# pythoncrazy/jimm

Hardware: NVIDIA H100
Metric: images/sec (higher is better)
Workload: dtype f16

## Files before the change

jimm_b200/csrc/common.cuh:

```cuda
#pragma once

#include <cuda.h>
#include <cuda_bf16.h>
#include <cuda_fp16.h>
#include <cuda_fp8.h>
#include <cuda_runtime.h>
#include <stdint.h>

#include <atomic>
#include <mutex>
#include <string>

namespace jimm {

void set_last_error(const char* fmt, ...);

#define JIMM_CUDA_CHECK(expr)                                                                   \
  do {                                                                                          \
    cudaError_t _e = (expr);                                                                    \
    if (_e != cudaSuccess) {                                                                    \
      ::jimm::set_last_error("%s:%d: %s -> %s", __FILE__, __LINE__, #expr, cudaGetErrorString(_e)); \
      return -2;                                                                                \
    }                                                                                           \
  } while (0)
// ... 80 lines not shown
      : "=r"(pred));
  return pred != 0;
}

__device__ __forceinline__ void mbar_init(uint64_t* bar, uint32_t count) {
  asm volatile("mbarrier.init.shared::cta.b64 [%0], %1;" ::"r"(smem_u32(bar)), "r"(count));
}
__device__ __forceinline__ void fence_barrier_init() {
  asm volatile("fence.mbarrier_init.release.cluster;" ::: "memory");
}
__device__ __forceinline__ void fence_proxy_async_smem() {
  asm volatile("fence.proxy.async.shared::cta;" ::: "memory");
}
__device__ __forceinline__ void mbar_arrive(uint64_t* bar) {
  asm volatile("mbarrier.arrive.shared::cta.b64 _, [%0];" ::"r"(smem_u32(bar)) : "memory");
}
__device__ __forceinline__ void mbar_arrive_expect_tx(uint64_t* bar, uint32_t bytes) {
  asm volatile("mbarrier.arrive.expect_tx.shared::cta.b64 _, [%0], %1;" ::"r"(smem_u32(bar)), "r"(bytes) : "memory");
}
__device__ __forceinline__ void mbar_wait(uint64_t* bar, uint32_t parity) {
  asm volatile(
      "{\n\t.reg .pred P1;\n\t"
      "WAIT_LOOP:\n\t"
      "mbarrier.try_wait.parity.shared::cta.b64 P1, [%0], %1;\n\t"
      "@P1 bra DONE;\n\t"
      "bra WAIT_LOOP;\n\t"
      "DONE:\n\t}" ::"r"(smem_u32(bar)),
      "r"(parity)
      : "memory");
}

__device__ __forceinline__ bool mbar_test_wait(uint64_t* bar, uint32_t parity) {
  uint32_t ok;
  asm volatile(
      "{\n\t.reg .pred P1;\n\t"
      "mbarrier.test_wait.parity.shared::cta.b64 P1, [%1], %2;\n\t"
      "selp.u32 %0, 1, 0, P1;\n\t}"
      : "=r"(ok)
      : "r"(smem_u32(bar)), "r"(parity)
      : "memory");
  return ok != 0;
}

__device__ __forceinline__ void tma_prefetch_desc(const CUtensorMap* m) {
  asm volatile("prefetch.tensormap [%0];" ::"l"(reinterpret_cast<uint64_t>(m)) : "memory");
}
__device__ __forceinline__ void tma_load_2d(void* smem_dst, const CUtensorMap* m, uint64_t* bar, int c0, int c1) {
  asm volatile(
      "cp.async.bulk.tensor.2d.shared::cluster.global.mbarrier::complete_tx::bytes [%0], [%1, {%3, %4}], [%2];" ::"r"(
          smem_u32(smem_dst)),
      "l"(reinterpret_cast<uint64_t>(m)), "r"(smem_u32(bar)), "r"(c0), "r"(c1)
      : "memory");
}

__device__ __forceinline__ void tma_store_2d(const CUtensorMap* m, uint32_t smem_src, int c0, int c1) {
  asm volatile("cp.async.bulk.tensor.2d.global.shared::cta.bulk_group [%0, {%2, %3}], [%1];" ::"l"(reinterpret_cast<uint64_t>(m)),
               "r"(smem_src), "r"(c0), "r"(c1)
               : "memory");
}
__device__ __forceinline__ void tma_reduce_add_2d(const CUtensorMap* m, uint32_t smem_src, int c0, int c1) {
  asm volatile("cp.reduce.async.bulk.tensor.2d.global.shared::cta.add.tile.bulk_group [%0, {%2, %3}], [%1];" ::"l"(
                   reinterpret_cast<uint64_t>(m)),
               "r"(smem_src), "r"(c0), "r"(c1)
               : "memory");
}
__device__ __forceinline__ void tma_store_3d(const CUtensorMap* m, uint32_t smem_src, int c0, int c1, int c2) {
  asm volatile("cp.async.bulk.tensor.3d.global.shared::cta.bulk_group [%0, {%2, %3, %4}], [%1];" ::"l"(reinterpret_cast<uint64_t>(m)),
               "r"(smem_src), "r"(c0), "r"(c1), "r"(c2)
               : "memory");
}
__device__ __forceinline__ void tma_reduce_add_3d(const CUtensorMap* m, uint32_t smem_src, int c0, int c1, int c2) {
  asm volatile("cp.reduce.async.bulk.tensor.3d.global.shared::cta.add.tile.bulk_group [%0, {%2, %3, %4}], [%1];" ::"l"(
                   reinterpret_cast<uint64_t>(m)),
               "r"(smem_src), "r"(c0), "r"(c1), "r"(c2)
               : "memory");
}
__device__ __forceinline__ void tma_store_commit() { asm volatile("cp.async.bulk.commit_group;" ::: "memory"); }
__device__ __forceinline__ void tma_store_wait_read() { asm volatile("cp.async.bulk.wait_group.read 0;" ::: "memory"); }
__device__ __forceinline__ void tma_store_wait_read1() { asm volatile("cp.async.bulk.wait_group.read 1;" ::: "memory"); }
__device__ __forceinline__ void tma_store_wait_all() { asm volatile("cp.async.bulk.wait_group 0;" ::: "memory"); }

__device__ __forceinline__ uint32_t cluster_ctarank() {
  uint32_t r;
  asm volatile("mov.u32 %0, %%cluster_ctarank;" : "=r"(r));
  return r;
}
__device__ __forceinline__ void cluster_sync_all() {
  asm volatile("barrier.cluster.arrive.release.aligned;\n\tbarrier.cluster.wait.acquire.aligned;" ::: "memory");
}
__device__ __forceinline__ uint32_t mapa_shared(uint32_t local_smem_addr, uint32_t rank) {
  uint32_t r;
  asm volatile("mapa.shared::cluster.u32 %0, %1, %2;" : "=r"(r) : "r"(local_smem_addr), "r"(rank));
  return r;
}
__device__ __forceinline__ void mbar_arrive_cluster(uint32_t cluster_addr) {
  asm volatile("mbarrier.arrive.release.cluster.shared::cluster.b64 _, [%0];" ::"r"(cluster_addr) : "memory");
}
__device__ __forceinline__ uint64_t make_wgmma_desc_sw128(uint32_t smem_addr) {
  uint64_t d = 0;
  d |= static_cast<uint64_t>((smem_addr & 0x3FFFFu) >> 4);
  d |= static_cast<uint64_t>(1) << 16;
  d |= static_cast<uint64_t>(1024 >> 4) << 32;
  d |= static_cast<uint64_t>(1) << 62;
  return d;
}
template <int SW>
__device__ __forceinline__ uint64_t make_wgmma_desc(uint32_t smem_addr, uint32_t lbo) {
  static_assert(SW == 128 || SW == 64 || SW == 32, "swizzle width");
  constexpr uint64_t layout = SW == 128 ? 1 : SW == 64 ? 2 : 3;
  uint64_t d = 0;
  d |= static_cast<uint64_t>((smem_addr & 0x3FFFFu) >> 4);
  d |= static_cast<uint64_t>((lbo >> 4) & 0x3FFFu) << 16;
  d |= static_cast<uint64_t>(8 * SW >> 4) << 32;
  d |= layout << 62;
  return d;
}
__device__ __forceinline__ void wgmma_fence() { asm volatile("wgmma.fence.sync.aligned;" ::: "memory"); }
__device__ __forceinline__ void wgmma_commit() { asm volatile("wgmma.commit_group.sync.aligned;" ::: "memory"); }
template <int N>
__device__ __forceinline__ void wgmma_wait() { asm volatile("wgmma.wait_group.sync.aligned %0;" ::"n"(N) : "memory"); }
template <int R>
__device__ __forceinline__ void wgmma_fence_operands(float (&d)[R]) {
#pragma unroll
  for (int i = 0; i < R; ++i) asm volatile("" : "+f"(d[i])::"memory");
}

#define JIMM_WGMMA_D128                                                                                                                    \
  "{%0, %1, %2, %3, %4, %5, %6, %7, %8, %9, %10, %11, %12, %13, %14, %15, %16, %17, %18, %19, %20, %21, %22, %23, %24, %25, %26, %27, "     \
  "%28, %29, %30, %31, %32, %33, %34, %35, %36, %37, %38, %39, %40, %41, %42, %43, %44, %45, %46, %47, %48, %49, %50, %51, %52, %53, %54, " \
  "%55, %56, %57, %58, %59, %60, %61, %62, %63, %64, %65, %66, %67, %68, %69, %70, %71, %72, %73, %74, %75, %76, %77, %78, %79, %80, %81, " \
  "%82, %83, %84, %85, %86, %87, %88, %89, %90, %91, %92, %93, %94, %95, %96, %97, %98, %99, %100, %101, %102, %103, %104, %105, %106, "   \
  "%107, %108, %109, %110, %111, %112, %113, %114, %115, %116, %117, %118, %119, %120, %121, %122, %123, %124, %125, %126, %127}"
#define JIMM_WGMMA_D8(i) "+f"(d[i]), "+f"(d[i + 1]), "+f"(d[i + 2]), "+f"(d[i + 3]), "+f"(d[i + 4]), "+f"(d[i + 5]), "+f"(d[i + 6]), "+f"(d[i + 7])
#define JIMM_WGMMA_D128_OPERANDS                                                                                                 \
  JIMM_WGMMA_D8(0), JIMM_WGMMA_D8(8), JIMM_WGMMA_D8(16), JIMM_WGMMA_D8(24), JIMM_WGMMA_D8(32), JIMM_WGMMA_D8(40), JIMM_WGMMA_D8(48), \
      JIMM_WGMMA_D8(56), JIMM_WGMMA_D8(64), JIMM_WGMMA_D8(72), JIMM_WGMMA_D8(80), JIMM_WGMMA_D8(88), JIMM_WGMMA_D8(96),             \
      JIMM_WGMMA_D8(104), JIMM_WGMMA_D8(112), JIMM_WGMMA_D8(120)
template <int KIND>
__device__ __forceinline__ void wgmma_m64n256_ss(float (&d)[128], uint64_t adesc, uint64_t bdesc, uint32_t accumulate) {
  if constexpr (KIND == 0) {
    asm volatile("{\n\t.reg .pred p;\n\tsetp.ne.b32 p, %130, 0;\n\t"
                 "wgmma.mma_async.sync.aligned.m64n256k16.f32.f16.f16 " JIMM_WGMMA_D128 ", %128, %129, p, 1, 1, 0, 0;\n\t}"
                 : JIMM_WGMMA_D128_OPERANDS
                 : "l"(adesc), "l"(bdesc), "r"(accumulate));
  } else if constexpr (KIND == 1) {
    asm volatile("{\n\t.reg .pred p;\n\tsetp.ne.b32 p, %130, 0;\n\t"
                 "wgmma.mma_async.sync.aligned.m64n256k16.f32.bf16.bf16 " JIMM_WGMMA_D128 ", %128, %129, p, 1, 1, 0, 0;\n\t}"
                 : JIMM_WGMMA_D128_OPERANDS
                 : "l"(adesc), "l"(bdesc), "r"(accumulate));
// ... 260 lines not shown
```

jimm_b200/csrc/gemm.cu:

```cuda
#include "gemm.cuh"

#include <stdarg.h>
#include <stdio.h>
#include <stdlib.h>
#include <string.h>

#include <type_traits>

#include "common.cuh"

namespace jimm {

static constexpr int BM = GEMM_TILE_M;
static constexpr int BN = GEMM_TILE_N;
static_assert(BM == 128 && BN == 256, "the warp roles and the wgmma shape below are written for 128 x 256 tiles");
static constexpr int STAGES = 4;
static constexpr int A_STAGE_BYTES = BM * 128;
static constexpr int B_STAGE_BYTES = BN * 128;
static constexpr int STAGE_BYTES = A_STAGE_BYTES + B_STAGE_BYTES;
static constexpr int EPI_WARPS = 8;
static constexpr int EPI_BOX_ROWS = 16;
static constexpr int EPI_BUF_BYTES = EPI_BOX_ROWS * 128;
static constexpr int EPI_BUFS = 2;
static constexpr int EPI_STAGE_BYTES = EPI_WARPS * EPI_BUFS * EPI_BUF_BYTES;
// ... 257 lines not shown
        *reinterpret_cast<float2*>(p1) = make_float2(v2, v3);
      }
    }
    fence_proxy_async_smem();
    __syncwarp();
    if (lane == 0) {
      const uint32_t tbuf_u32 = smem_u32(tbuf);
      if constexpr (OUT == OUT_F32_ADD) {
        if (epi.tok_pad > 0) {
          const int b = row_base / epi.tok_pad;
          tma_reduce_add_3d(map_c, tbuf_u32, n0, row_base - b * epi.tok_pad + epi.tok_off, b);
        } else {
          tma_reduce_add_2d(map_c, tbuf_u32, n0, row_base);
        }
      } else {
        tma_store_2d(map_c, tbuf_u32, n0, row_base);
      }
      tma_store_commit();
    }
  }
}

template <bool SCALED, int NC>
__device__ __forceinline__ void epilogue_generic(const EpiDev& epi, const float (&acc)[NC / 2], int lane, int row_base, int n_tile0) {
  const int g = lane >> 2, t = lane & 3;
#pragma unroll
  for (int h = 0; h < 2; ++h) {
    const int row = row_base + g + 8 * h;
    if (row >= epi.M) continue;
    int out_row, add_row;
    remap_row(epi, row, out_row, add_row);
    float sa = 1.f;
    if constexpr (SCALED) sa = __ldg(epi.a_scale + row);
#pragma unroll
    for (int j = 0; j < NC / 8; ++j) {
#pragma unroll
      for (int q = 0; q < 2; ++q) {
        const int col = n_tile0 + 8 * j + 2 * t + q;
        if (col < epi.N) {
          float v = acc[4 * j + 2 * h + q];
          if constexpr (SCALED) v *= sa * __ldg(epi.b_scale + col);
          if (epi.bias) v += __ldg(epi.bias + col);
          v = apply_act(v, epi.act);
          if (epi.rowadd) v += __ldg(epi.rowadd + static_cast<size_t>(add_row) * epi.N + col);
          if (epi.residual) v += epi.residual[static_cast<size_t>(out_row) * epi.ldr + col];
          store1(epi, out_row, col, v);
        }
      }
    }
  }
}


template <typename T, int OUT, int ACT>
__global__ void __launch_bounds__(NUM_THREADS, 1)
gemm_wgmma_kernel(const __grid_constant__ CUtensorMap map_a, const __grid_constant__ CUtensorMap map_b,
                  const __grid_constant__ CUtensorMap map_c, const EpiDev epi, int K) {
  constexpr bool SCALED = kScaled<T>;
  constexpr int BK = 128 / sizeof(T);
  constexpr int UK = 32 / sizeof(T);
  constexpr int TM = tile_rows(Traits<T>::DTYPE);
  constexpr int STAGE_TX = TM * 128 + B_STAGE_BYTES;
  constexpr int WG_DM = SCALED ? 0 : 64;
  constexpr int WG_DN = SCALED ? 128 : 0;
  constexpr int NC = BN - WG_DN;
  constexpr bool FUSE_LN = OUT == OUT_F32_ADD && ACT == ACT_FUSE_LN;
  constexpr int EPI_ACT = ACT == ACT_FUSE_LN ? static_cast<int>(ACT_NONE) : ACT;
  constexpr int PRODUCER_REGS = FUSE_LN ? 152 : 40;
  constexpr int CONSUMER_REGS = FUSE_LN ? 176 : 232;
  static_assert(128 * PRODUCER_REGS + 256 * CONSUMER_REGS <= NUM_THREADS * KERNEL_REGS, "register split exceeds the CTA's allocation");

  extern __shared__ uint8_t smem_raw[];
  uint8_t* smem = reinterpret_cast<uint8_t*>((reinterpret_cast<uintptr_t>(smem_raw) + 1023) & ~static_cast<uintptr_t>(1023));
  uint8_t* smem_a = smem;
  uint8_t* smem_b = smem + STAGES * A_STAGE_BYTES;
  uint8_t* epi_stage = smem + STAGES * STAGE_BYTES;
  LnQueue* lnq = reinterpret_cast<LnQueue*>(epi_stage + EPI_STAGE_BYTES);
  uint64_t* full_bar = reinterpret_cast<uint64_t*>(lnq + 1);
  uint64_t* empty_bar = full_bar + STAGES;

  const int warp_idx = threadIdx.x >> 5;
  const int lane = threadIdx.x & 31;
  const int M = epi.M, N = epi.N;
  const int m_tiles = (M + TM - 1) / TM, n_tiles = (N + BN - 1) / BN;
  const int num_tiles = m_tiles * n_tiles;
  const int num_kb = (K + BK - 1) / BK;

  pdl_launch_dependents();
  if (warp_idx == 0 && lane == 0) {
    tma_prefetch_desc(&map_a);
    tma_prefetch_desc(&map_b);
    if constexpr (OUT != OUT_GENERIC) tma_prefetch_desc(&map_c);
    for (int s = 0; s < STAGES; ++s) {
      mbar_init(&full_bar[s], 1);
      mbar_init(&empty_bar[s], EPI_WARPS);
    }
    fence_barrier_init();
  }
  if constexpr (FUSE_LN) {
    if (warp_idx == 1) {
      for (int i = lane; i < LNQ; i += 32) lnq->slot[i] = -1;
      if (lane == 0) lnq->head = lnq->tail = lnq->done = 0;
    }
  }
  __syncthreads();
  pdl_wait();

  if (warp_idx < 4) {
    setmaxnreg<KERNEL_REGS, PRODUCER_REGS>();
    if (warp_idx == 0) {
      if (lane == 0) {
        int stage = 0;
        uint32_t phase = 0;
        for (int tile = blockIdx.x; tile < num_tiles; tile += gridDim.x) {
          const int tv = epi.reverse ? num_tiles - 1 - tile : tile;
          const int m_blk = tv / n_tiles, n_blk = tv - m_blk * n_tiles;
          for (int kb = 0; kb < num_kb; ++kb) {
            mbar_wait(&empty_bar[stage], phase ^ 1);
            mbar_arrive_expect_tx(&full_bar[stage], STAGE_TX);
            tma_load_2d(smem_a + stage * A_STAGE_BYTES, &map_a, &full_bar[stage], kb * BK, m_blk * TM);
            tma_load_2d(smem_b + stage * B_STAGE_BYTES, &map_b, &full_bar[stage], kb * BK, n_blk * BN);
            if (++stage == STAGES) { stage = 0; phase ^= 1; }
          }
        }
      }
    } else if constexpr (FUSE_LN) {
      ln_worker<T>(epi, lnq, lane);
    }
  } else {
    setmaxnreg<KERNEL_REGS, CONSUMER_REGS>();
    const int wg = (warp_idx - 4) >> 2;
    const int wq = warp_idx & 3;
    uint8_t* tbuf0 = epi_stage + (warp_idx - 4) * EPI_BUFS * EPI_BUF_BYTES;
    int stage = 0;
    uint32_t phase = 0, box_count = 0;
    int ln_rg = -1, ln_cols = 0;
    float acc[NC / 2];
    for (int tile = blockIdx.x; tile < num_tiles; tile += gridDim.x) {
      const int tv = epi.reverse ? num_tiles - 1 - tile : tile;
      const int m_blk = tv / n_tiles, n_blk = tv - m_blk * n_tiles;
      int prev = -1;
      if constexpr (SCALED) {
#pragma unroll
        for (int i = 0; i < NC / 2; ++i) acc[i] = 0.f;
      }
      for (int kb = 0; kb < num_kb; ++kb) {
        mbar_wait(&full_bar[stage], phase);
        const uint64_t adesc = make_wgmma_desc_sw128(smem_u32(smem_a + stage * A_STAGE_BYTES + wg * WG_DM * 128));
        const uint64_t bdesc = make_wgmma_desc_sw128(smem_u32(smem_b + stage * B_STAGE_BYTES + wg * WG_DN * 128));
        if constexpr (SCALED) {
          float slab[NC / 2];
          wgmma_fence_operands(slab);
          wgmma_fence();
#pragma unroll
          for (int k = 0; k < BK / UK; ++k)
            wgmma_m64n128k32_e4m3_ss(slab, adesc + static_cast<uint64_t>(2 * k), bdesc + static_cast<uint64_t>(2 * k), k != 0 ? 1u : 0u);
          wgmma_commit();
          wgmma_wait<0>();
          wgmma_fence_operands(slab);
          if (lane == 0) mbar_arrive(&empty_bar[stage]);
#pragma unroll
          for (int i = 0; i < NC / 2; ++i) acc[i] += slab[i];
        } else {
          wgmma_fence_operands(acc);
          wgmma_fence();
#pragma unroll
          for (int k = 0; k < BK / UK; ++k)
            wgmma_m64n256_ss<Traits<T>::KIND>(acc, adesc + static_cast<uint64_t>(2 * k), bdesc + static_cast<uint64_t>(2 * k), (kb | k) != 0 ? 1u : 0u);
          wgmma_commit();
          wgmma_fence_operands(acc);
          if (prev >= 0) {
            wgmma_wait<1>();
            if (lane == 0) mbar_arrive(&empty_bar[prev]);
          }
          prev = stage;
        }
        if (++stage == STAGES) { stage = 0; phase ^= 1; }
      }
      if constexpr (!SCALED) {
        wgmma_wait<0>();
        wgmma_fence_operands(acc);
        if (lane == 0) mbar_arrive(&empty_bar[prev]);
      }

      const int row_base = m_blk * TM + wg * WG_DM + wq * 16;
      const int n_tile0 = n_blk * BN + wg * WG_DN;
      if constexpr (OUT == OUT_GENERIC) {
        epilogue_generic<SCALED, NC>(epi, acc, lane, row_base, n_tile0);
      } else {
        if (row_base < M && (WG_DN == 0 || n_tile0 < N))
          epilogue_tma<OUT, EPI_ACT, SCALED, NC>(&map_c, epi, acc, tbuf0, lane, row_base, n_tile0, box_count);
        if constexpr (FUSE_LN) {
          if (lane == 0 && ln_rg >= 0) ln_publish(epi, lnq, ln_rg, ln_cols);
          ln_rg = (row_base & ~31) < M ? row_base >> 5 : -1;
          ln_cols = min(BN, N - n_tile0);
        }
      }
    }
    if constexpr (FUSE_LN) {
      if (lane == 0) {
        if (ln_rg >= 0) ln_publish(epi, lnq, ln_rg, ln_cols);
        __threadfence_block();
        atomicAdd(&lnq->done, 1);
      }
    }
    if constexpr (OUT != OUT_GENERIC) {
      if (lane == 0) tma_store_wait_all();
    }
  }
}

template <typename T>
__global__ void gemm_simt_kernel(const T* __restrict__ A, int lda, const T* __restrict__ B, int ldb, int K, EpiDev epi) {
  __shared__ float As[16][17], Bs[16][17];
  const int tx = threadIdx.x, ty = threadIdx.y;
  const int row = blockIdx.y * 16 + ty, col = blockIdx.x * 16 + tx;
  float acc = 0.f;
  for (int k0 = 0; k0 < K; k0 += 16) {
    const int ar = blockIdx.y * 16 + ty, ak = k0 + tx;
    As[ty][tx] = (ar < epi.M && ak < K) ? to_float(A[static_cast<size_t>(ar) * lda + ak]) : 0.f;
    const int br = blockIdx.x * 16 + ty, bk = k0 + tx;
    Bs[ty][tx] = (br < epi.N && bk < K) ? to_float(B[static_cast<size_t>(br) * ldb + bk]) : 0.f;
    __syncthreads();
#pragma unroll
    for (int k = 0; k < 16; ++k) acc += As[ty][k] * Bs[tx][k];
    __syncthreads();
  }
  if (row < epi.M && col < epi.N) {
    int out_row, add_row;
    remap_row(epi, row, out_row, add_row);
    float v = acc;
    if constexpr (kScaled<T>) v *= epi.a_scale[row] * epi.b_scale[col];
    if (epi.bias) v += epi.bias[col];
    v = apply_act(v, epi.act);
    if (epi.rowadd) v += epi.rowadd[static_cast<size_t>(add_row) * epi.N + col];
    if (epi.residual) v += epi.residual[static_cast<size_t>(out_row) * epi.ldr + col];
    store1(epi, out_row, col, v);
  }
}

static constexpr int SMEM_BYTES = STAGES * STAGE_BYTES + EPI_STAGE_BYTES + static_cast<int>(sizeof(LnQueue)) + 2 * STAGES * 8 + 1024;
static_assert(SMEM_BYTES <= 232448, "exceeds 227 KB of shared memory");
typedef CUresult (*PFN_encodeTiled)(CUtensorMap*, CUtensorMapDataType, cuuint32_t, void*, const cuuint64_t*, const cuuint64_t*,
                                    const cuuint32_t*, const cuuint32_t*, CUtensorMapInterleave, CUtensorMapSwizzle,
                                    CUtensorMapL2promotion, CUtensorMapFloatOOBfill);

static PFN_encodeTiled get_encode_fn() {
  static std::atomic<PFN_encodeTiled> fn{nullptr};
  if (PFN_encodeTiled f = fn.load(std::memory_order_acquire)) return f;
  void* p = nullptr;
  cudaDriverEntryPointQueryResult qres;
  cudaError_t e = cudaGetDriverEntryPoint("cuTensorMapEncodeTiled", &p, cudaEnableDefault, &qres);
  if (e != cudaSuccess || qres != cudaDriverEntryPointSuccess || p == nullptr) {
    set_last_error("cudaGetDriverEntryPoint(cuTensorMapEncodeTiled) failed: %s", cudaGetErrorString(e));
    return nullptr;
  }
  fn.store(reinterpret_cast<PFN_encodeTiled>(p), std::memory_order_release);
  return reinterpret_cast<PFN_encodeTiled>(p);
}

static CUtensorMapDataType tensor_map_dtype(int dtype) {
  switch (dtype) {
// ... 40 lines not shown
  return 0;
}

int device_sm_count() {
  static std::atomic<int> sms[DeviceOnce::kMaxDevices] = {};
  int dev = 0;
  cudaGetDevice(&dev);
  if (dev < 0 || dev >= DeviceOnce::kMaxDevices) dev = 0;
  int n = sms[dev].load(std::memory_order_relaxed);
  if (n == 0) {
    cudaDeviceGetAttribute(&n, cudaDevAttrMultiProcessorCount, dev);
    const char* env = getenv("JIMM_NUM_SMS");
    if (env && atoi(env) > 0) n = atoi(env);
    sms[dev].store(n, std::memory_order_relaxed);
  }
  return n;
}

static int check_epi(const GemmEpilogue& e, int N) {
  if (e.out == nullptr) { set_last_error("gemm: null output"); return -1; }
  if (e.ldo < N) { set_last_error("gemm: ldo (%d) < N (%d)", e.ldo, N); return -1; }
  return 0;
}
static int check_e4m3_epi(const GemmEpilogue& e) {
  if (e.a_scale == nullptr || e.b_scale == nullptr) { set_last_error("gemm: e4m3 operands need row scales for A and B"); return -1; }
  if ((reinterpret_cast<uintptr_t>(e.b_scale) & 7) != 0) { set_last_error("gemm: the B scales must be 8-byte aligned"); return -1; }
  if (e.residual || e.rowadd || e.rows_in != 0 || e.tok_pad != 0 || e.ln_cnt) {
    set_last_error("gemm: e4m3 operands support bias and activation epilogues only (no residual, row-add, row remap, token scatter or "
                   "fused LayerNorm)");
    return -1;
  }
  return 0;
}
int gemm_plan_init(GemmPlan* plan, int dtype, const void* A, int lda, const void* B, int ldb, int M, int N, int K,
                   const GemmEpilogue& epi) {
  if (M <= 0 || N <= 0 || K <= 0) { set_last_error("gemm: bad shape %dx%dx%d", M, N, K); return -1; }
  if (int rc = check_epi(epi, N)) return rc;
  if (dtype == DT_E4M3) {
    if (int rc = check_e4m3_epi(epi)) return rc;
  }
  if (epi.tok_pad != 0) {
    if (epi.tok_pad < 0 || epi.tok_pad % EPI_BOX_ROWS != 0 || M % epi.tok_pad != 0 || epi.tok_off < 0 || epi.tok_S <= 0) {
      set_last_error("gemm: token scatter needs tok_pad a positive multiple of %d dividing M (tok_pad=%d M=%d tok_off=%d tok_S=%d)", EPI_BOX_ROWS,
                     epi.tok_pad, M, epi.tok_off, epi.tok_S);
      return -1;
    }
    if (epi.residual != epi.out || epi.ldr != epi.ldo || epi.out_type != DT_F32) {
      set_last_error("gemm: token scatter reduce-adds into an fp32 output that is also the residual");
      return -1;
    }
  }
  if (int rc = make_tensor_map_2d(&plan->map_a, dtype, A, M, K, lda, tile_rows(dtype))) return rc;
  if (int rc = make_tensor_map_2d(&plan->map_b, dtype, B, N, K, ldb, BN)) return rc;
  plan->M = M; plan->N = N; plan->K = K; plan->dtype = dtype; plan->epi = epi;
  memset(&plan->map_c, 0, sizeof(plan->map_c));
  if (plan->epi.mode == 2) {
    const size_t es = dtype_size(epi.out_type);
    const bool ok = epi.rowadd == nullptr && epi.rows_in == 0 && (static_cast<size_t>(N) * es) % 16 == 0 &&
                    (epi.residual == nullptr || (epi.residual == epi.out && epi.ldr == epi.ldo && epi.out_type == DT_F32)) &&
                    (static_cast<size_t>(epi.ldo) * es) % 16 == 0 && (reinterpret_cast<uintptr_t>(epi.out) & 15) == 0 &&
                    (epi.bias == nullptr || ((reinterpret_cast<uintptr_t>(epi.bias) & 15) == 0 && N % 4 == 0)) &&
                    !(epi.residual && epi.act != ACT_NONE);
    if (ok && epi.tok_pad > 0) {
      if (int rc = make_tensor_map_3d(&plan->map_c, DT_F32, epi.out, M / epi.tok_pad, epi.tok_S, N, epi.ldo)) return rc;
    } else if (ok) {
      if (int rc = make_tensor_map_2d(&plan->map_c, epi.out_type, epi.out, M, N, epi.ldo, EPI_BOX_ROWS)) return rc;
    } else {
      plan->epi.mode = 0;
    }
  }
  if (epi.tok_pad > 0 && plan->epi.mode != 2) {
    set_last_error("gemm: the token scatter needs the TMA epilogue (mode 2, no activation, 16-byte aligned output / bias, N %% 4 == 0)");
    return -1;
  }
  return 0;
}

static EpiDev to_dev(const GemmEpilogue& e, int M, int N) {
  EpiDev d;
  d.bias = e.bias; d.rowadd = e.rowadd; d.residual = e.residual; d.out = e.out;
  d.act = e.act; d.ldr = e.ldr; d.out_type = e.out_type; d.ldo = e.ldo;
  d.rows_in = e.rows_in; d.rows_out = e.rows_out; d.row_off = e.row_off; d.mode = e.mode;
  d.M = M; d.N = N;
  d.tok_pad = e.tok_pad; d.tok_off = e.tok_off;
  d.reverse = e.reverse;
  d.ln_scale = e.ln_scale; d.ln_bias = e.ln_bias; d.ln_out = e.ln_out; d.ln_cnt = e.ln_cnt;
  d.ln_out_type = e.ln_out_type; d.ln_ldo = e.ln_ldo; d.ln_eps = e.ln_eps;
  d.a_scale = e.a_scale; d.b_scale = e.b_scale;
  return d;
}

template <typename T, int OUT, int ACT>
static int launch_one(const GemmPlan* p, int M, cudaStream_t stream) {
  auto* kernel = gemm_wgmma_kernel<T, OUT, ACT>;
  constexpr int TM = tile_rows(Traits<T>::DTYPE);
  static DeviceOnce attr_set;
  if (int rc = attr_set.run([&]() -> int {
        JIMM_CUDA_CHECK(cudaFuncSetAttribute(kernel, cudaFuncAttributeMaxDynamicSharedMemorySize, SMEM_BYTES));
        cudaFuncAttributes fa;
        JIMM_CUDA_CHECK(cudaFuncGetAttributes(&fa, kernel));
        if (fa.numRegs != KERNEL_REGS) {
          set_last_error("gemm: kernel compiled with %d registers per thread, the warpgroup register split assumes %d", fa.numRegs, KERNEL_REGS);
          return -2;
        }
        return 0;
      }))
    return rc;
  const int tiles = ((M + TM - 1) / TM) * ((p->N + BN - 1) / BN);
  const int grid = tiles < device_sm_count() ? tiles : device_sm_count();
  JIMM_CUDA_CHECK(launch_k(kernel, dim3(grid), dim3(NUM_THREADS), SMEM_BYTES, stream, 1, true, p->map_a, p->map_b, p->map_c,
                           to_dev(p->epi, M, p->N), p->K));
  note_launch();
  return 0;
}

template <typename T, int OUT>
static int launch_act(const GemmPlan* p, int M, cudaStream_t stream) {
  switch (p->epi.act) {
    case ACT_GELU_TANH: return launch_one<T, OUT, ACT_GELU_TANH>(p, M, stream);
    case ACT_QUICK_GELU: return launch_one<T, OUT, ACT_QUICK_GELU>(p, M, stream);
    default: return launch_one<T, OUT, ACT_NONE>(p, M, stream);
  }
}

template <typename T>
static int launch_tc(const GemmPlan* p, int M, cudaStream_t stream) {
  const GemmEpilogue& e = p->epi;
  if (e.mode != 2) return launch_one<T, OUT_GENERIC, ACT_NONE>(p, M, stream);
  if constexpr (!kScaled<T>) {
    if (e.residual) return gemm_fuses_ln(p, M) ? launch_one<T, OUT_F32_ADD, ACT_FUSE_LN>(p, M, stream) : launch_one<T, OUT_F32_ADD, ACT_NONE>(p, M, stream);
  }
  switch (e.out_type) {
    case DT_F16: return launch_act<T, OUT_H16>(p, M, stream);
    case DT_BF16: return launch_act<T, OUT_BF16>(p, M, stream);
    case DT_TF32: return launch_act<T, OUT_TF32>(p, M, stream);
    default: return launch_act<T, OUT_F32>(p, M, stream);
  }
}

int gemm_fuses_ln(const GemmPlan* p, int ) {
  const int nv = p->N >> 7;
  const bool width_ok = p->N % 128 == 0 && (nv <= 4 || nv == 6 || nv == 8 || nv == 9);
  const int want = p->dtype == DT_F16 ? DT_F16 : p->dtype == DT_BF16 ? DT_BF16 : DT_TF32;
  return p->epi.ln_cnt != nullptr && p->epi.ln_out_type == want && width_ok && p->epi.mode == 2 && p->epi.residual != nullptr && p->epi.tok_pad == 0;
}

int gemm_plan_run(const GemmPlan* p0, int M_override, cudaStream_t stream, int reverse) {
  const int M = (M_override > 0 && M_override <= p0->M) ? M_override : p0->M;
  if (p0->epi.tok_pad > 0 && M % p0->epi.tok_pad != 0) {
    set_last_error("gemm: token scatter runs whole samples (M=%d, tok_pad=%d)", M, p0->epi.tok_pad);
    return -1;
  }
  GemmPlan local;
  const GemmPlan* p = p0;
  if (reverse != p0->epi.reverse) { local = *p0; local.epi.reverse = reverse; p = &local; }
  switch (p->dtype) {
    case DT_F16: return launch_tc<__half>(p, M, stream);
    case DT_BF16: return launch_tc<__nv_bfloat16>(p, M, stream);
    case DT_F32:
    case DT_TF32: return launch_tc<float>(p, M, stream);
    case DT_E4M3: return launch_tc<__nv_fp8_e4m3>(p, M, stream);
  }
  set_last_error("gemm: bad dtype %d", p->dtype);
  return -1;
}

int gemm_simt_run(int dtype, const void* A, int lda, const void* B, int ldb, int M, int N, int K, const GemmEpilogue& epi,
                  cudaStream_t stream) {
  if (int rc = check_epi(epi, N)) return rc;
  if (dtype == DT_E4M3) {
    if (int rc = check_e4m3_epi(epi)) return rc;
  }
  dim3 block(16, 16), grid((N + 15) / 16, (M + 15) / 16);
  EpiDev d = to_dev(epi, M, N);
  if (dtype == DT_F16) gemm_simt_kernel<__half><<<grid, block, 0, stream>>>(static_cast<const __half*>(A), lda, static_cast<const __half*>(B), ldb, K, d);
  else if (dtype == DT_BF16) gemm_simt_kernel<__nv_bfloat16><<<grid, block, 0, stream>>>(static_cast<const __nv_bfloat16*>(A), lda, static_cast<const __nv_bfloat16*>(B), ldb, K, d);
  else if (dtype == DT_E4M3) gemm_simt_kernel<__nv_fp8_e4m3><<<grid, block, 0, stream>>>(static_cast<const __nv_fp8_e4m3*>(A), lda, static_cast<const __nv_fp8_e4m3*>(B), ldb, K, d);
  else gemm_simt_kernel<float><<<grid, block, 0, stream>>>(static_cast<const float*>(A), lda, static_cast<const float*>(B), ldb, K, d);
  JIMM_LAUNCH_CHECK();
  return 0;
}

}
```

jimm_b200/csrc/gemm.cuh:

```cuda
#pragma once
#include <cuda.h>
#include <cuda_runtime.h>
#include <stdint.h>

namespace jimm {

enum DType : int { DT_F32 = 0, DT_F16 = 1, DT_BF16 = 2, DT_TF32 = 3, DT_E4M3 = 4 };
enum Act : int { ACT_NONE = 0, ACT_GELU_TANH = 1, ACT_QUICK_GELU = 2 };

inline size_t dtype_size(int dt) { return (dt == DT_F32 || dt == DT_TF32) ? 4 : dt == DT_E4M3 ? 1 : 2; }

constexpr int GEMM_TILE_M = 128;
constexpr int GEMM_TILE_N = 256;

struct GemmEpilogue {
  const float* bias = nullptr;
  int act = ACT_NONE;
  const float* rowadd = nullptr;
  const float* residual = nullptr;
  int ldr = 0;
  void* out = nullptr;
  int out_type = DT_F32;
  int ldo = 0;
  int tok_pad = 0, tok_off = 0, tok_S = 0;
  int reverse = 0;
  int rows_in = 0, rows_out = 0, row_off = 0;
  int mode = 2;
  const float* ln_scale = nullptr;
  const float* ln_bias = nullptr;
  void* ln_out = nullptr;
  int ln_out_type = DT_F16, ln_ldo = 0;
  float ln_eps = 1e-6f;
  int* ln_cnt = nullptr;
  const float* a_scale = nullptr;
  const float* b_scale = nullptr;
};

struct GemmPlan {
  CUtensorMap map_a, map_b, map_c;
  int M = 0, N = 0, K = 0;
  int dtype = DT_F16;
  GemmEpilogue epi;
};

int gemm_plan_init(GemmPlan* plan, int dtype, const void* A, int lda, const void* B, int ldb, int M, int N, int K,
                   const GemmEpilogue& epi);
int gemm_plan_run(const GemmPlan* plan, int M_override, cudaStream_t stream, int reverse = 0);

int gemm_simt_run(int dtype, const void* A, int lda, const void* B, int ldb, int M, int N, int K, const GemmEpilogue& epi,
                  cudaStream_t stream);

int gemm_fuses_ln(const GemmPlan* plan, int M_override);

int device_sm_count();

}
```

jimm_b200/csrc/kernel_api.cu:

```cuda
#include <mutex>

#include "../../include/jimm_b200.h"
#include "common.cuh"
#include "gemm.cuh"
#include "kernels.cuh"

namespace jimm {
extern std::mutex g_capture_mu;
}

using namespace jimm;

extern "C" {

int jimm_k_gemm_ex(int impl, int dtype, const void* A, int lda, const void* B, int ldb, int M, int N, int K, const float* bias, int act,
                   const float* rowadd, const float* residual, int ldr, void* out, int out_type, int ldo, int rows_in, int rows_out,
                   int row_off, int epi_mode, int plan_M, int reverse, int tok_pad, int tok_off, int tok_S, const float* ln_scale,
                   const float* ln_bias, float ln_eps, void* ln_out, int ln_out_type, int ln_ldo, int* ln_counters, void* stream) {
  if (plan_M <= 0) plan_M = M;
  if (M <= 0 || M > plan_M) { set_last_error("jimm_k_gemm_ex: need 0 < M <= plan_M (M=%d plan_M=%d)", M, plan_M); return JIMM_EINVAL; }
  GemmEpilogue e;
  e.bias = bias; e.act = act; e.rowadd = rowadd; e.residual = residual; e.ldr = ldr; e.out = out; e.out_type = out_type; e.ldo = ldo;
  e.rows_in = rows_in; e.rows_out = rows_out; e.row_off = row_off; e.mode = epi_mode;
  e.tok_pad = tok_pad; e.tok_off = tok_off; e.tok_S = tok_S;
  if (ln_counters) {
    e.ln_scale = ln_scale; e.ln_bias = ln_bias; e.ln_out = ln_out; e.ln_out_type = ln_out_type == JIMM_F32 ? DT_TF32 : ln_out_type; e.ln_ldo = ln_ldo;
    e.ln_eps = ln_eps; e.ln_cnt = ln_counters;
  }
  cudaStream_t s = static_cast<cudaStream_t>(stream);
  if (impl == 1) {
    if (plan_M != M || reverse || tok_pad || ln_counters) {
      set_last_error("jimm_k_gemm_ex: the SIMT GEMM has no plan rows, reverse walk, token scatter or fused LayerNorm");
      return JIMM_EINVAL;
    }
    return gemm_simt_run(dtype, A, lda, B, ldb, M, N, K, e, s);
  }
  GemmPlan p;
  if (int rc = gemm_plan_init(&p, dtype, A, lda, B, ldb, plan_M, N, K, e)) return rc;
  if (ln_counters && !gemm_fuses_ln(&p, M)) {
    set_last_error("gemm: this shape does not take the fused LayerNorm path (needs N = 128 x {1,2,3,4,6,8,9}, aligned operands, "
                   "LayerNorm output in the operand type)");
    return JIMM_EINVAL;
  }
  return gemm_plan_run(&p, M, s, reverse);
}
int jimm_k_gemm(int impl, int dtype, const void* A, int lda, const void* B, int ldb, int M, int N, int K, const float* bias, int act,
                const float* rowadd, const float* residual, int ldr, void* out, int out_type, int ldo, int rows_in, int rows_out,
                int row_off, int epi_mode, void* stream) {
  return jimm_k_gemm_ex(impl, dtype, A, lda, B, ldb, M, N, K, bias, act, rowadd, residual, ldr, out, out_type, ldo, rows_in, rows_out, row_off,
                        epi_mode, M, 0, 0, 0, 0, nullptr, nullptr, 0.f, nullptr, 0, 0, nullptr, stream);
}
int jimm_k_gemm_residual_ln(int dtype, const void* A, int lda, const void* B, int ldb, int M, int N, int K, const float* bias, float* x, int ldx,
                            const float* ln_scale, const float* ln_bias, float eps, void* ln_out, int ln_out_type, int ln_ldo, int* counters,
                            void* stream) {
  if (!counters) { set_last_error("jimm_k_gemm_residual_ln: null counters"); return JIMM_EINVAL; }
  return jimm_k_gemm_ex(0, dtype, A, lda, B, ldb, M, N, K, bias, 0, nullptr, x, ldx, x, JIMM_F32, ldx, 0, 0, 0, 2, M, 0, 0, 0, 0, ln_scale,
                        ln_bias, eps, ln_out, ln_out_type, ln_ldo, counters, stream);
}
int jimm_k_layernorm_ex(const float* x, int ldx, int group, int row_off, const int32_t* row_index, const float* scale, const float* bias,
                        float eps, void* out, int out_type, int ldy, int rows, int D, int reverse, void* stream) {
  return layernorm_run(x, ldx, group, row_off, row_index, scale, bias, eps, out, out_type, ldy, rows, D, static_cast<cudaStream_t>(stream), reverse);
}
int jimm_k_layernorm(const float* x, int ldx, int group, int row_off, const int32_t* row_index, const float* scale, const float* bias,
                     float eps, void* out, int out_type, int ldy, int rows, int D, void* stream) {
  return jimm_k_layernorm_ex(x, ldx, group, row_off, row_index, scale, bias, eps, out, out_type, ldy, rows, D, 0, stream);
}
int jimm_k_layernorm_e4m3(const float* x, int ldx, const float* scale, const float* bias, float eps, void* out, int ldy, float* row_scale,
                          int rows, int D, int reverse, void* stream) {
  return layernorm_run(x, ldx, 1, 0, nullptr, scale, bias, eps, out, DT_E4M3, ldy, rows, D, static_cast<cudaStream_t>(stream), reverse,
                       row_scale);
}
int jimm_k_gemm_e4m3(int impl, const void* A, int lda, const void* B, int ldb, int M, int N, int K, const float* a_scale, const float* b_scale,
                     const float* bias, int act, void* out, int out_type, int ldo, int epi_mode, int plan_M, int reverse, void* stream) {
  if (plan_M <= 0) plan_M = M;
  if (M <= 0 || M > plan_M) { set_last_error("jimm_k_gemm_e4m3: need 0 < M <= plan_M (M=%d plan_M=%d)", M, plan_M); return JIMM_EINVAL; }
  if (out_type < DT_F32 || out_type > DT_TF32) { set_last_error("jimm_k_gemm_e4m3: bad output type %d", out_type); return JIMM_EINVAL; }
  GemmEpilogue e;
  e.bias = bias; e.act = act; e.out = out; e.out_type = out_type; e.ldo = ldo; e.mode = epi_mode;
  e.a_scale = a_scale; e.b_scale = b_scale;
  cudaStream_t s = static_cast<cudaStream_t>(stream);
  if (impl == 1) {
    if (plan_M != M || reverse) { set_last_error("jimm_k_gemm_e4m3: the SIMT GEMM has no plan rows or reverse walk"); return JIMM_EINVAL; }
    return gemm_simt_run(DT_E4M3, A, lda, B, ldb, M, N, K, e, s);
  }
  GemmPlan p;
  if (int rc = gemm_plan_init(&p, DT_E4M3, A, lda, B, ldb, plan_M, N, K, e)) return rc;
  return gemm_plan_run(&p, M, s, reverse);
}
int jimm_k_quantize_e4m3(const float* src, int lds, int rows, int K, void* out, int ldo, float* row_scale, void* stream) {
  return quantize_rows_e4m3_run(src, lds, rows, K, out, ldo, row_scale, static_cast<cudaStream_t>(stream));
}
int jimm_k_attention_hd(const void* qkv, int io_type, void* out, int out_type, int B, int S, int H, int head_dim, int causal, int reverse,
                        void* stream) {
  return attention_run(qkv, io_type, out, out_type, B, S, H, head_dim, causal, static_cast<cudaStream_t>(stream), reverse);
}
int jimm_k_attention_ex(const void* qkv, int io_type, void* out, int out_type, int B, int S, int H, int causal, int reverse, void* stream) {
  return jimm_k_attention_hd(qkv, io_type, out, out_type, B, S, H, 64, causal, reverse, stream);
// ... 95 lines not shown
```

jimm_b200/csrc/probe.cu:

```cuda
#include "../../include/jimm_b200.h"
#include "common.cuh"
#include "gemm.cuh"

namespace jimm {

int make_tensor_map_2d(CUtensorMap* map, int dtype, const void* ptr, int rows, int cols, int ld, int box_rows);

namespace {

constexpr int PB_STAGES = 12;
constexpr int PB_STAGE_BYTES = 128 * 128;

__device__ __forceinline__ void tma_load_2d_multicast(void* smem_dst, const CUtensorMap* m, uint64_t* bar, int c0, int c1, uint16_t mask) {
  asm volatile(
      "cp.async.bulk.tensor.2d.shared::cluster.global.mbarrier::complete_tx::bytes.multicast::cluster [%0], [%1, {%3, %4}], [%2], %5;" ::"r"(
          smem_u32(smem_dst)),
      "l"(reinterpret_cast<uint64_t>(m)), "r"(smem_u32(bar)), "r"(c0), "r"(c1), "h"(mask)
      : "memory");
}

template <int CS>
__global__ void __launch_bounds__(64, 1) l2_probe_kernel(const __grid_constant__ CUtensorMap map_full, const __grid_constant__ CUtensorMap map_part,
                                                         int mode, int iters, int total_rows) {
  extern __shared__ uint8_t smem_raw[];
  uint8_t* smem = reinterpret_cast<uint8_t*>((reinterpret_cast<uintptr_t>(smem_raw) + 1023) & ~static_cast<uintptr_t>(1023));
  uint64_t* full = reinterpret_cast<uint64_t*>(smem + PB_STAGES * PB_STAGE_BYTES);
  uint64_t* empty = full + PB_STAGES;
  const uint32_t rank = CS > 1 ? cluster_ctarank() : 0;
  const int cluster_id = blockIdx.x / CS;
  const bool shared_writes = CS > 1 && mode == 2;
  if (threadIdx.x == 0) {
    for (int i = 0; i < PB_STAGES; ++i) {
      mbar_init(&full[i], 1);
      mbar_init(&empty[i], shared_writes ? CS : 1);
    }
    fence_barrier_init();
  }
  __syncthreads();
  if (CS > 1) cluster_sync_all();
  const int tiles = total_rows / 128;
  if (threadIdx.x == 0) {
    int st = 0;
    uint32_t ph = 0;
    for (int it = 0; it < iters; ++it) {
      const long long tile = mode == 0 ? (static_cast<long long>(blockIdx.x) * iters + it) : (static_cast<long long>(cluster_id) * iters + it);
      const int row = static_cast<int>((tile * 7919) % tiles) * 128;
      mbar_wait(&empty[st], ph ^ 1);
      mbar_arrive_expect_tx(&full[st], PB_STAGE_BYTES);
      if (mode == 2 && CS > 1) {
        constexpr int part = 128 / CS;
        tma_load_2d_multicast(smem + st * PB_STAGE_BYTES + rank * part * 128, &map_part, &full[st], 0, row + rank * part,
                              static_cast<uint16_t>((1u << CS) - 1));
      } else {
        tma_load_2d(smem + st * PB_STAGE_BYTES, &map_full, &full[st], 0, row);
      }
      if (++st == PB_STAGES) { st = 0; ph ^= 1; }
    }
  } else if (threadIdx.x == 32) {
    int st = 0;
    uint32_t ph = 0;
    for (int it = 0; it < iters; ++it) {
      mbar_wait(&full[st], ph);
      if (shared_writes) {
        for (uint32_t r = 0; r < CS; ++r)
          asm volatile("mbarrier.arrive.relaxed.cluster.shared::cluster.b64 _, [%0];" ::"r"(mapa_shared(smem_u32(&empty[st]), r)) : "memory");
      } else {
        mbar_arrive(&empty[st]);
      }
      if (++st == PB_STAGES) { st = 0; ph ^= 1; }
    }
  }
  __syncthreads();
// ... 48 lines not shown
```

Baseline: 12170.

## Pair CTAs in clusters of two and multicast the shared B tile

The persistent wgmma GEMM now runs 16-bit GEMMs as 2-CTA clusters along M. Each CTA loads half of the shared 256-wide B tile through TMA multicast to both CTAs, so B traffic from L2 is halved. Stage release now arrives on the peer CTA's empty barrier as well, and each cluster must fit within the occupancy limit. The cost is cross-CTA coupling: a stage can only be reused once both consumers finish, and there are extra cluster syncs at start and end.

```diff
diff --git a/jimm_b200/csrc/common.cuh b/jimm_b200/csrc/common.cuh
--- a/jimm_b200/csrc/common.cuh
+++ b/jimm_b200/csrc/common.cuh
@@ -156,6 +156,13 @@
       "l"(reinterpret_cast<uint64_t>(m)), "r"(smem_u32(bar)), "r"(c0), "r"(c1)
       : "memory");
 }
+__device__ __forceinline__ void tma_load_2d_multicast(void* smem_dst, const CUtensorMap* m, uint64_t* bar, int c0, int c1, uint16_t mask) {
+  asm volatile(
+      "cp.async.bulk.tensor.2d.shared::cluster.global.mbarrier::complete_tx::bytes.multicast::cluster [%0], [%1, {%3, %4}], [%2], %5;" ::"r"(
+          smem_u32(smem_dst)),
+      "l"(reinterpret_cast<uint64_t>(m)), "r"(smem_u32(bar)), "r"(c0), "r"(c1), "h"(mask)
+      : "memory");
+}
 
 __device__ __forceinline__ void tma_store_2d(const CUtensorMap* m, uint32_t smem_src, int c0, int c1) {
   asm volatile("cp.async.bulk.tensor.2d.global.shared::cta.bulk_group [%0, {%2, %3}], [%1];" ::"l"(reinterpret_cast<uint64_t>(m)),
@@ -199,6 +206,9 @@
 }
 __device__ __forceinline__ void mbar_arrive_cluster(uint32_t cluster_addr) {
   asm volatile("mbarrier.arrive.release.cluster.shared::cluster.b64 _, [%0];" ::"r"(cluster_addr) : "memory");
+}
+__device__ __forceinline__ void mbar_arrive_peer(uint32_t cluster_addr) {
+  asm volatile("mbarrier.arrive.shared::cluster.b64 _, [%0];" ::"r"(cluster_addr) : "memory");
 }
 __device__ __forceinline__ uint64_t make_wgmma_desc_sw128(uint32_t smem_addr) {
   uint64_t d = 0;
diff --git a/jimm_b200/csrc/gemm.cu b/jimm_b200/csrc/gemm.cu
--- a/jimm_b200/csrc/gemm.cu
+++ b/jimm_b200/csrc/gemm.cu
@@ -333,11 +333,12 @@
 }
 
 
-template <typename T, int OUT, int ACT>
+template <typename T, int OUT, int ACT, int CS>
 __global__ void __launch_bounds__(NUM_THREADS, 1)
 gemm_wgmma_kernel(const __grid_constant__ CUtensorMap map_a, const __grid_constant__ CUtensorMap map_b,
                   const __grid_constant__ CUtensorMap map_c, const EpiDev epi, int K) {
   constexpr bool SCALED = kScaled<T>;
+  static_assert(CS == 1 || (CS == GEMM_CLUSTER_M && !SCALED), "CTA pairs split the B tile of the 16-bit / tf32 slab body");
   constexpr int BK = 128 / sizeof(T);
   constexpr int UK = 32 / sizeof(T);
   constexpr int TM = tile_rows(Traits<T>::DTYPE);
@@ -364,7 +365,9 @@
   const int lane = threadIdx.x & 31;
   const int M = epi.M, N = epi.N;
   const int m_tiles = (M + TM - 1) / TM, n_tiles = (N + BN - 1) / BN;
-  const int num_tiles = m_tiles * n_tiles;
+  const int num_tiles = (m_tiles + CS - 1) / CS * n_tiles;
+  const int first_tile = blockIdx.x / CS, tile_step = gridDim.x / CS;
+  const int rank = CS > 1 ? static_cast<int>(cluster_ctarank()) : 0;
   const int num_kb = (K + BK - 1) / BK;
 
   pdl_launch_dependents();
@@ -374,7 +377,7 @@
     if constexpr (OUT != OUT_GENERIC) tma_prefetch_desc(&map_c);
     for (int s = 0; s < STAGES; ++s) {
       mbar_init(&full_bar[s], 1);
-      mbar_init(&empty_bar[s], EPI_WARPS);
+      mbar_init(&empty_bar[s], CS * EPI_WARPS);
     }
     fence_barrier_init();
   }
@@ -385,6 +388,7 @@
     }
   }
   __syncthreads();
+  if constexpr (CS > 1) cluster_sync_all();
   pdl_wait();
 
   if (warp_idx < 4) {
@@ -393,14 +397,21 @@
       if (lane == 0) {
         int stage = 0;
         uint32_t phase = 0;
-        for (int tile = blockIdx.x; tile < num_tiles; tile += gridDim.x) {
+        for (int tile = first_tile; tile < num_tiles; tile += tile_step) {
           const int tv = epi.reverse ? num_tiles - 1 - tile : tile;
-          const int m_blk = tv / n_tiles, n_blk = tv - m_blk * n_tiles;
+          const int m_grp = tv / n_tiles, n_blk = tv - m_grp * n_tiles;
+          const int m_blk = m_grp * CS + rank;
           for (int kb = 0; kb < num_kb; ++kb) {
             mbar_wait(&empty_bar[stage], phase ^ 1);
             mbar_arrive_expect_tx(&full_bar[stage], STAGE_TX);
             tma_load_2d(smem_a + stage * A_STAGE_BYTES, &map_a, &full_bar[stage], kb * BK, m_blk * TM);
-            tma_load_2d(smem_b + stage * B_STAGE_BYTES, &map_b, &full_bar[stage], kb * BK, n_blk * BN);
+            if constexpr (CS == 1) {
+              tma_load_2d(smem_b + stage * B_STAGE_BYTES, &map_b, &full_bar[stage], kb * BK, n_blk * BN);
+            } else {
+              constexpr int PART = BN / CS;
+              tma_load_2d_multicast(smem_b + stage * B_STAGE_BYTES + rank * PART * 128, &map_b, &full_bar[stage], kb * BK,
+                                    n_blk * BN + rank * PART, static_cast<uint16_t>((1u << CS) - 1));
+            }
             if (++stage == STAGES) { stage = 0; phase ^= 1; }
           }
         }
@@ -417,9 +428,19 @@
     uint32_t phase = 0, box_count = 0;
     int ln_rg = -1, ln_cols = 0;
     float acc[NC / 2];
-    for (int tile = blockIdx.x; tile < num_tiles; tile += gridDim.x) {
+    auto release = [&](int s) {
+      if (lane != 0) return;
+      mbar_arrive(&empty_bar[s]);
+      if constexpr (CS > 1) {
+#pragma unroll
+        for (int r = 0; r < CS; ++r)
+          if (r != rank) mbar_arrive_peer(mapa_shared(smem_u32(&empty_bar[s]), static_cast<uint32_t>(r)));
+      }
+    };
+    for (int tile = first_tile; tile < num_tiles; tile += tile_step) {
       const int tv = epi.reverse ? num_tiles - 1 - tile : tile;
-      const int m_blk = tv / n_tiles, n_blk = tv - m_blk * n_tiles;
+      const int m_grp = tv / n_tiles, n_blk = tv - m_grp * n_tiles;
+      const int m_blk = m_grp * CS + rank;
       int prev = -1;
       if constexpr (SCALED) {
 #pragma unroll
@@ -439,7 +460,7 @@
           wgmma_commit();
           wgmma_wait<0>();
           wgmma_fence_operands(slab);
-          if (lane == 0) mbar_arrive(&empty_bar[stage]);
+          release(stage);
 #pragma unroll
           for (int i = 0; i < NC / 2; ++i) acc[i] += slab[i];
         } else {
@@ -452,7 +473,7 @@
           wgmma_fence_operands(acc);
           if (prev >= 0) {
             wgmma_wait<1>();
-            if (lane == 0) mbar_arrive(&empty_bar[prev]);
+            release(prev);
           }
           prev = stage;
         }
@@ -461,7 +482,7 @@
       if constexpr (!SCALED) {
         wgmma_wait<0>();
         wgmma_fence_operands(acc);
-        if (lane == 0) mbar_arrive(&empty_bar[prev]);
+        release(prev);
       }
 
       const int row_base = m_blk * TM + wg * WG_DM + wq * 16;
@@ -489,6 +510,10 @@
       if (lane == 0) tma_store_wait_all();
     }
   }
+  if constexpr (CS > 1) {
+    __syncwarp();
+    cluster_sync_all();
+  }
 }
 
 template <typename T>
@@ -635,6 +660,10 @@
   }
   if (int rc = make_tensor_map_2d(&plan->map_a, dtype, A, M, K, lda, tile_rows(dtype))) return rc;
   if (int rc = make_tensor_map_2d(&plan->map_b, dtype, B, N, K, ldb, BN)) return rc;
+  memset(&plan->map_b_half, 0, sizeof(plan->map_b_half));
+  if (dtype == DT_F16 || dtype == DT_BF16) {
+    if (int rc = make_tensor_map_2d(&plan->map_b_half, dtype, B, N, K, ldb, BN / GEMM_CLUSTER_M)) return rc;
+  }
   plan->M = M; plan->N = N; plan->K = K; plan->dtype = dtype; plan->epi = epi;
   memset(&plan->map_c, 0, sizeof(plan->map_c));
   if (plan->epi.mode == 2) {
@@ -673,11 +702,15 @@
   return d;
 }
 
-template <typename T, int OUT, int ACT>
-static int launch_one(const GemmPlan* p, int M, cudaStream_t stream) {
-  auto* kernel = gemm_wgmma_kernel<T, OUT, ACT>;
+template <typename T, int OUT, int ACT, int CS>
+static int launch_cs(const GemmPlan* p, int M, cudaStream_t stream) {
+  auto* kernel = gemm_wgmma_kernel<T, OUT, ACT, CS>;
   constexpr int TM = tile_rows(Traits<T>::DTYPE);
   static DeviceOnce attr_set;
+  static int max_clusters[DeviceOnce::kMaxDevices];
+  int dev = 0;
+  cudaGetDevice(&dev);
+  if (dev < 0 || dev >= DeviceOnce::kMaxDevices) dev = 0;
   if (int rc = attr_set.run([&]() -> int {
         JIMM_CUDA_CHECK(cudaFuncSetAttribute(kernel, cudaFuncAttributeMaxDynamicSharedMemorySize, SMEM_BYTES));
         cudaFuncAttributes fa;
@@ -686,38 +719,70 @@
           set_last_error("gemm: kernel compiled with %d registers per thread, the warpgroup register split assumes %d", fa.numRegs, KERNEL_REGS);
           return -2;
         }
+        if constexpr (CS > 1) {
+          cudaLaunchConfig_t cfg = {};
+          cudaLaunchAttribute attr;
+          attr.id = cudaLaunchAttributeClusterDimension;
+          attr.val.clusterDim.x = CS;
+          attr.val.clusterDim.y = 1;
+          attr.val.clusterDim.z = 1;
+          cfg.gridDim = dim3(CS);
+          cfg.blockDim = dim3(NUM_THREADS);
+          cfg.dynamicSmemBytes = SMEM_BYTES;
+          cfg.attrs = &attr;
+          cfg.numAttrs = 1;
+          int n = 0;
+          JIMM_CUDA_CHECK(cudaOccupancyMaxActiveClusters(&n, kernel, &cfg));
+          if (n <= 0) {
+            set_last_error("gemm: no cluster of %d CTAs with %d bytes of shared memory fits on this device", CS, SMEM_BYTES);
+            return -2;
+          }
+          max_clusters[dev] = n;
+        }
         return 0;
       }))
     return rc;
-  const int tiles = ((M + TM - 1) / TM) * ((p->N + BN - 1) / BN);
-  const int grid = tiles < device_sm_count() ? tiles : device_sm_count();
-  JIMM_CUDA_CHECK(launch_k(kernel, dim3(grid), dim3(NUM_THREADS), SMEM_BYTES, stream, 1, true, p->map_a, p->map_b, p->map_c,
-                           to_dev(p->epi, M, p->N), p->K));
+  const int tiles = ((M + TM * CS - 1) / (TM * CS)) * ((p->N + BN - 1) / BN);
+  int slots = device_sm_count() / CS;
+  if (CS > 1 && max_clusters[dev] < slots) slots = max_clusters[dev];
+  const int grid = CS * (tiles < slots ? tiles : slots);
+  JIMM_CUDA_CHECK(launch_k(kernel, dim3(grid), dim3(NUM_THREADS), SMEM_BYTES, stream, CS, true, p->map_a, CS > 1 ? p->map_b_half : p->map_b,
+                           p->map_c, to_dev(p->epi, M, p->N), p->K));
   note_launch();
   return 0;
 }
 
+template <typename T, int OUT, int ACT>
+static int launch_one(const GemmPlan* p, int M, cudaStream_t stream, int pair) {
+  constexpr bool PAIRED = sizeof(T) == 2 && (OUT == OUT_H16 || OUT == OUT_BF16 || OUT == OUT_F32_ADD || OUT == OUT_F32);
+  if constexpr (PAIRED) {
+    if (pair && M > tile_rows(Traits<T>::DTYPE)) return launch_cs<T, OUT, ACT, GEMM_CLUSTER_M>(p, M, stream);
+  }
+  return launch_cs<T, OUT, ACT, 1>(p, M, stream);
+}
+
 template <typename T, int OUT>
-static int launch_act(const GemmPlan* p, int M, cudaStream_t stream) {
+static int launch_act(const GemmPlan* p, int M, cudaStream_t stream, int pair) {
   switch (p->epi.act) {
-    case ACT_GELU_TANH: return launch_one<T, OUT, ACT_GELU_TANH>(p, M, stream);
-    case ACT_QUICK_GELU: return launch_one<T, OUT, ACT_QUICK_GELU>(p, M, stream);
-    default: return launch_one<T, OUT, ACT_NONE>(p, M, stream);
+    case ACT_GELU_TANH: return launch_one<T, OUT, ACT_GELU_TANH>(p, M, stream, pair);
+    case ACT_QUICK_GELU: return launch_one<T, OUT, ACT_QUICK_GELU>(p, M, stream, pair);
+    default: return launch_one<T, OUT, ACT_NONE>(p, M, stream, pair);
   }
 }
 
 template <typename T>
-static int launch_tc(const GemmPlan* p, int M, cudaStream_t stream) {
+static int launch_tc(const GemmPlan* p, int M, cudaStream_t stream, int pair) {
   const GemmEpilogue& e = p->epi;
-  if (e.mode != 2) return launch_one<T, OUT_GENERIC, ACT_NONE>(p, M, stream);
+  if (e.mode != 2) return launch_one<T, OUT_GENERIC, ACT_NONE>(p, M, stream, pair);
   if constexpr (!kScaled<T>) {
-    if (e.residual) return gemm_fuses_ln(p, M) ? launch_one<T, OUT_F32_ADD, ACT_FUSE_LN>(p, M, stream) : launch_one<T, OUT_F32_ADD, ACT_NONE>(p, M, stream);
+    if (e.residual)
+      return gemm_fuses_ln(p, M) ? launch_one<T, OUT_F32_ADD, ACT_FUSE_LN>(p, M, stream, pair) : launch_one<T, OUT_F32_ADD, ACT_NONE>(p, M, stream, pair);
   }
   switch (e.out_type) {
-    case DT_F16: return launch_act<T, OUT_H16>(p, M, stream);
-    case DT_BF16: return launch_act<T, OUT_BF16>(p, M, stream);
-    case DT_TF32: return launch_act<T, OUT_TF32>(p, M, stream);
-    default: return launch_act<T, OUT_F32>(p, M, stream);
+    case DT_F16: return launch_act<T, OUT_H16>(p, M, stream, pair);
+    case DT_BF16: return launch_act<T, OUT_BF16>(p, M, stream, pair);
+    case DT_TF32: return launch_act<T, OUT_TF32>(p, M, stream, pair);
+    default: return launch_act<T, OUT_F32>(p, M, stream, pair);
   }
 }
 
@@ -728,7 +793,7 @@
   return p->epi.ln_cnt != nullptr && p->epi.ln_out_type == want && width_ok && p->epi.mode == 2 && p->epi.residual != nullptr && p->epi.tok_pad == 0;
 }
 
-int gemm_plan_run(const GemmPlan* p0, int M_override, cudaStream_t stream, int reverse) {
+int gemm_plan_run(const GemmPlan* p0, int M_override, cudaStream_t stream, int reverse, int pair) {
   const int M = (M_override > 0 && M_override <= p0->M) ? M_override : p0->M;
   if (p0->epi.tok_pad > 0 && M % p0->epi.tok_pad != 0) {
     set_last_error("gemm: token scatter runs whole samples (M=%d, tok_pad=%d)", M, p0->epi.tok_pad);
@@ -738,11 +803,11 @@
   const GemmPlan* p = p0;
   if (reverse != p0->epi.reverse) { local = *p0; local.epi.reverse = reverse; p = &local; }
   switch (p->dtype) {
-    case DT_F16: return launch_tc<__half>(p, M, stream);
-    case DT_BF16: return launch_tc<__nv_bfloat16>(p, M, stream);
+    case DT_F16: return launch_tc<__half>(p, M, stream, pair);
+    case DT_BF16: return launch_tc<__nv_bfloat16>(p, M, stream, pair);
     case DT_F32:
-    case DT_TF32: return launch_tc<float>(p, M, stream);
-    case DT_E4M3: return launch_tc<__nv_fp8_e4m3>(p, M, stream);
+    case DT_TF32: return launch_tc<float>(p, M, stream, pair);
+    case DT_E4M3: return launch_tc<__nv_fp8_e4m3>(p, M, stream, pair);
   }
   set_last_error("gemm: bad dtype %d", p->dtype);
   return -1;
diff --git a/jimm_b200/csrc/gemm.cuh b/jimm_b200/csrc/gemm.cuh
--- a/jimm_b200/csrc/gemm.cuh
+++ b/jimm_b200/csrc/gemm.cuh
@@ -12,6 +12,7 @@
 
 constexpr int GEMM_TILE_M = 128;
 constexpr int GEMM_TILE_N = 256;
+constexpr int GEMM_CLUSTER_M = 2;
 
 struct GemmEpilogue {
   const float* bias = nullptr;
@@ -38,6 +39,7 @@
 
 struct GemmPlan {
   CUtensorMap map_a, map_b, map_c;
+  CUtensorMap map_b_half;
   int M = 0, N = 0, K = 0;
   int dtype = DT_F16;
   GemmEpilogue epi;
@@ -45,7 +47,7 @@
 
 int gemm_plan_init(GemmPlan* plan, int dtype, const void* A, int lda, const void* B, int ldb, int M, int N, int K,
                    const GemmEpilogue& epi);
-int gemm_plan_run(const GemmPlan* plan, int M_override, cudaStream_t stream, int reverse = 0);
+int gemm_plan_run(const GemmPlan* plan, int M_override, cudaStream_t stream, int reverse = 0, int pair = 1);
 
 int gemm_simt_run(int dtype, const void* A, int lda, const void* B, int ldb, int M, int N, int K, const GemmEpilogue& epi,
                   cudaStream_t stream);
diff --git a/jimm_b200/csrc/kernel_api.cu b/jimm_b200/csrc/kernel_api.cu
--- a/jimm_b200/csrc/kernel_api.cu
+++ b/jimm_b200/csrc/kernel_api.cu
@@ -42,7 +42,7 @@
                    "LayerNorm output in the operand type)");
     return JIMM_EINVAL;
   }
-  return gemm_plan_run(&p, M, s, reverse);
+  return gemm_plan_run(&p, M, s, reverse, impl == 2 ? 0 : 1);
 }
 int jimm_k_gemm(int impl, int dtype, const void* A, int lda, const void* B, int ldb, int M, int N, int K, const float* bias, int act,
                 const float* rowadd, const float* residual, int ldr, void* out, int out_type, int ldo, int rows_in, int rows_out,
diff --git a/jimm_b200/csrc/probe.cu b/jimm_b200/csrc/probe.cu
--- a/jimm_b200/csrc/probe.cu
+++ b/jimm_b200/csrc/probe.cu
@@ -10,14 +10,6 @@
 
 constexpr int PB_STAGES = 12;
 constexpr int PB_STAGE_BYTES = 128 * 128;
-
-__device__ __forceinline__ void tma_load_2d_multicast(void* smem_dst, const CUtensorMap* m, uint64_t* bar, int c0, int c1, uint16_t mask) {
-  asm volatile(
-      "cp.async.bulk.tensor.2d.shared::cluster.global.mbarrier::complete_tx::bytes.multicast::cluster [%0], [%1, {%3, %4}], [%2], %5;" ::"r"(
-          smem_u32(smem_dst)),
-      "l"(reinterpret_cast<uint64_t>(m)), "r"(smem_u32(bar)), "r"(c0), "r"(c1), "h"(mask)
-      : "memory");
-}
 
 template <int CS>
 __global__ void __launch_bounds__(64, 1) l2_probe_kernel(const __grid_constant__ CUtensorMap map_full, const __grid_constant__ CUtensorMap map_part,
```

Result: no change. 12260 (median of 6 runs) (+0.7%).
